# ZhengyiLuo/PHC

Measured on NVIDIA H100. Metric: env-steps/sec (fused obs+reward+PPO) at 4096 envs/GPU, higher is better.
Workload: dtype f32

## Files before the change

phc_b200/csrc/gemm_wgmma.cu:

```cuda
#include <cuda_runtime.h>
#include <stdint.h>
#include <stdlib.h>
#include <string.h>

#include "../../include/phc_b200.h"
#include "phc_common.cuh"

extern "C" void phc_set_error(const char* msg);
extern "C" int phc_check_cuda(cudaError_t e, const char* what);
extern "C" void phc_count_launches(int n);

namespace phc {
namespace wg {

constexpr int BM = 128, NUM_THREADS = 256, MAX_PROBLEMS = PHC_GEMM_GROUP_MAX;

template <int BN>
struct Cfg {
  static constexpr int BK = BN == 128 ? 32 : 16;
  static constexpr int A_TILE = BM * BK * 4;
  static constexpr int B_TILE = BN * BK * 4;
  static constexpr int STAGE = 2 * (A_TILE + B_TILE);
  static constexpr int SMEM = 2 * STAGE;
  static constexpr int SBO = BK * 32;
  static constexpr int A_PER = BM * BK / NUM_THREADS;
  static constexpr int B_PER = BN * BK / NUM_THREADS;
};

struct Prob {
  const float* A; const float* B; const float* A_lo; const float* B_lo;
  float* C; float* C_hi; float* C_lo;
  const float* bias;
  float* aux;
  long long lda, ldb, ldc, ldaux;
  int M, N, K;
  float alpha;
  int act, accumulate, a_k, b_k, k_splits;
  int tiles_m, tiles_n, kb_total, kb_per, tile_begin, tile_count;
  unsigned int* turn;
  int turn_first, turn_total;
};

struct Params {
  Prob p[MAX_PROBLEMS];
  int count, total_tiles;
  unsigned int* sched;
  int single_pass;
};

__device__ __forceinline__ void wgmma_tf32_n128(float (&d)[64], uint64_t da, uint64_t db) {
  asm volatile(
      "{\n\t.reg .pred p;\n\tsetp.ne.b32 p, 1, 0;\n\t"
      "wgmma.mma_async.sync.aligned.m64n128k8.f32.tf32.tf32 {%0, %1, %2, %3, %4, %5, %6, %7, %8, %9, %10, %11, %12, %13, %14, %15, %16, %17, %18, %19, %20, %21, %22, %23, %24, %25, %26, %27, %28, %29, %30, %31, %32, %33, %34, %35, %36, %37, %38, %39, %40, %41, %42, %43, %44, %45, %46, %47, %48, %49, %50, %51, %52, %53, %54, %55, %56, %57, %58, %59, %60, %61, %62, %63}, %64, %65, p, 1, 1;\n\t}"
      : "+f"(d[0]), "+f"(d[1]), "+f"(d[2]), "+f"(d[3]), "+f"(d[4]), "+f"(d[5]), "+f"(d[6]), "+f"(d[7]), "+f"(d[8]), "+f"(d[9]), "+f"(d[10]), "+f"(d[11]), "+f"(d[12]), "+f"(d[13]), "+f"(d[14]), "+f"(d[15]), "+f"(d[16]), "+f"(d[17]), "+f"(d[18]), "+f"(d[19]), "+f"(d[20]), "+f"(d[21]), "+f"(d[22]), "+f"(d[23]), "+f"(d[24]), "+f"(d[25]), "+f"(d[26]), "+f"(d[27]), "+f"(d[28]), "+f"(d[29]), "+f"(d[30]), "+f"(d[31]), "+f"(d[32]), "+f"(d[33]), "+f"(d[34]), "+f"(d[35]), "+f"(d[36]), "+f"(d[37]), "+f"(d[38]), "+f"(d[39]), "+f"(d[40]), "+f"(d[41]), "+f"(d[42]), "+f"(d[43]), "+f"(d[44]), "+f"(d[45]), "+f"(d[46]), "+f"(d[47]), "+f"(d[48]), "+f"(d[49]), "+f"(d[50]), "+f"(d[51]), "+f"(d[52]), "+f"(d[53]), "+f"(d[54]), "+f"(d[55]), "+f"(d[56]), "+f"(d[57]), "+f"(d[58]), "+f"(d[59]), "+f"(d[60]), "+f"(d[61]), "+f"(d[62]), "+f"(d[63])
      : "l"(da), "l"(db));
}
__device__ __forceinline__ void wgmma_tf32_n256(float (&d)[128], uint64_t da, uint64_t db) {
  asm volatile(
      "{\n\t.reg .pred p;\n\tsetp.ne.b32 p, 1, 0;\n\t"
      "wgmma.mma_async.sync.aligned.m64n256k8.f32.tf32.tf32 {%0, %1, %2, %3, %4, %5, %6, %7, %8, %9, %10, %11, %12, %13, %14, %15, %16, %17, %18, %19, %20, %21, %22, %23, %24, %25, %26, %27, %28, %29, %30, %31, %32, %33, %34, %35, %36, %37, %38, %39, %40, %41, %42, %43, %44, %45, %46, %47, %48, %49, %50, %51, %52, %53, %54, %55, %56, %57, %58, %59, %60, %61, %62, %63, %64, %65, %66, %67, %68, %69, %70, %71, %72, %73, %74, %75, %76, %77, %78, %79, %80, %81, %82, %83, %84, %85, %86, %87, %88, %89, %90, %91, %92, %93, %94, %95, %96, %97, %98, %99, %100, %101, %102, %103, %104, %105, %106, %107, %108, %109, %110, %111, %112, %113, %114, %115, %116, %117, %118, %119, %120, %121, %122, %123, %124, %125, %126, %127}, %128, %129, p, 1, 1;\n\t}"
      : "+f"(d[0]), "+f"(d[1]), "+f"(d[2]), "+f"(d[3]), "+f"(d[4]), "+f"(d[5]), "+f"(d[6]), "+f"(d[7]), "+f"(d[8]), "+f"(d[9]), "+f"(d[10]), "+f"(d[11]), "+f"(d[12]), "+f"(d[13]), "+f"(d[14]), "+f"(d[15]), "+f"(d[16]), "+f"(d[17]), "+f"(d[18]), "+f"(d[19]), "+f"(d[20]), "+f"(d[21]), "+f"(d[22]), "+f"(d[23]), "+f"(d[24]), "+f"(d[25]), "+f"(d[26]), "+f"(d[27]), "+f"(d[28]), "+f"(d[29]), "+f"(d[30]), "+f"(d[31]), "+f"(d[32]), "+f"(d[33]), "+f"(d[34]), "+f"(d[35]), "+f"(d[36]), "+f"(d[37]), "+f"(d[38]), "+f"(d[39]), "+f"(d[40]), "+f"(d[41]), "+f"(d[42]), "+f"(d[43]), "+f"(d[44]), "+f"(d[45]), "+f"(d[46]), "+f"(d[47]), "+f"(d[48]), "+f"(d[49]), "+f"(d[50]), "+f"(d[51]), "+f"(d[52]), "+f"(d[53]), "+f"(d[54]), "+f"(d[55]), "+f"(d[56]), "+f"(d[57]), "+f"(d[58]), "+f"(d[59]), "+f"(d[60]), "+f"(d[61]), "+f"(d[62]), "+f"(d[63]), "+f"(d[64]), "+f"(d[65]), "+f"(d[66]), "+f"(d[67]), "+f"(d[68]), "+f"(d[69]), "+f"(d[70]), "+f"(d[71]), "+f"(d[72]), "+f"(d[73]), "+f"(d[74]), "+f"(d[75]), "+f"(d[76]), "+f"(d[77]), "+f"(d[78]), "+f"(d[79]), "+f"(d[80]), "+f"(d[81]), "+f"(d[82]), "+f"(d[83]), "+f"(d[84]), "+f"(d[85]), "+f"(d[86]), "+f"(d[87]), "+f"(d[88]), "+f"(d[89]), "+f"(d[90]), "+f"(d[91]), "+f"(d[92]), "+f"(d[93]), "+f"(d[94]), "+f"(d[95]), "+f"(d[96]), "+f"(d[97]), "+f"(d[98]), "+f"(d[99]), "+f"(d[100]), "+f"(d[101]), "+f"(d[102]), "+f"(d[103]), "+f"(d[104]), "+f"(d[105]), "+f"(d[106]), "+f"(d[107]), "+f"(d[108]), "+f"(d[109]), "+f"(d[110]), "+f"(d[111]), "+f"(d[112]), "+f"(d[113]), "+f"(d[114]), "+f"(d[115]), "+f"(d[116]), "+f"(d[117]), "+f"(d[118]), "+f"(d[119]), "+f"(d[120]), "+f"(d[121]), "+f"(d[122]), "+f"(d[123]), "+f"(d[124]), "+f"(d[125]), "+f"(d[126]), "+f"(d[127])
      : "l"(da), "l"(db));
}

__device__ __forceinline__ void wgmma_fence() { asm volatile("wgmma.fence.sync.aligned;" ::: "memory"); }
__device__ __forceinline__ void wgmma_commit() { asm volatile("wgmma.commit_group.sync.aligned;" ::: "memory"); }
__device__ __forceinline__ void wgmma_wait_all() { asm volatile("wgmma.wait_group.sync.aligned 0;" ::: "memory"); }

__device__ __forceinline__ uint64_t smem_desc(uint32_t addr, uint32_t lbo, uint32_t sbo) {
  return (uint64_t)((addr & 0x3FFFF) >> 4) | ((uint64_t)(lbo >> 4) << 16) | ((uint64_t)(sbo >> 4) << 32);
}

template <int BN, typename Acc>
__device__ __forceinline__ void wgmma_tf32(Acc& d, uint64_t da, uint64_t db) {
  if constexpr (BN == 128) wgmma_tf32_n128(d, da, db); else wgmma_tf32_n256(d, da, db);
}

__device__ __forceinline__ float trunc_hi(float x) { return __uint_as_float(__float_as_uint(x) & 0xFFFFE000u); }
__device__ __forceinline__ float split_lo(float x) {
  const float d = x - trunc_hi(x);
  return __uint_as_float((__float_as_uint(d) + 0x1000u) & 0xFFFFE000u);
}
__device__ __forceinline__ void sts128(uint32_t addr, float a, float b, float c, float d) {
  asm volatile("st.shared.v4.f32 [%0], {%1, %2, %3, %4};" ::"r"(addr), "f"(a), "f"(b), "f"(c), "f"(d) : "memory");
}
__device__ __forceinline__ void sts32(uint32_t addr, float a) { asm volatile("st.shared.f32 [%0], %1;" ::"r"(addr), "f"(a) : "memory"); }

template <int R, int BK>
struct Map {
  static constexpr int KC = BK / 4;
  __device__ static void kmaj(int c, int& r, int& kc) { r = (c & 7) + 8 * (c / (8 * KC)); kc = (c >> 3) % KC; }
  __device__ static void mnmaj(int e, int& r, int& k, uint32_t& off) {
    const int rl = e & 7, kl = (e >> 3) & 3, e2 = e >> 5, rh = e2 % (R / 8), kh = e2 / (R / 8);
    r = rh * 8 + rl; k = kh * 4 + kl;
    off = (uint32_t)(rh * BK * 32 + kh * 128 + rl * 16 + kl * 4);
  }
};

template <int R, int BK, int PER>
__device__ __forceinline__ void load_op(float (&v)[PER], const float* __restrict__ g, long long ld, bool kmaj, int r0, int rows, int k0,
                                        int K, int tid) {
  using Mp = Map<R, BK>;
  if (kmaj) {
#pragma unroll
    for (int i = 0; i < PER / 4; ++i) {
      int r, kc;
      Mp::kmaj(tid + i * NUM_THREADS, r, kc);
      const int rr = r0 + r, kk = k0 + 4 * kc;
      const float* src = g + (long long)rr * ld + kk;
      if (rr < rows && kk + 3 < K) {
        const float4 t = *reinterpret_cast<const float4*>(src);
        v[4 * i] = t.x; v[4 * i + 1] = t.y; v[4 * i + 2] = t.z; v[4 * i + 3] = t.w;
      } else {
#pragma unroll
        for (int e = 0; e < 4; ++e) v[4 * i + e] = (rr < rows && kk + e < K) ? src[e] : 0.f;
      }
    }
  } else {
#pragma unroll
    for (int i = 0; i < PER; ++i) {
      int r, k;
      uint32_t off;
      Mp::mnmaj(tid + i * NUM_THREADS, r, k, off);
      const int rr = r0 + r, kk = k0 + k;
      v[i] = (rr < rows && kk < K) ? g[(long long)kk * ld + rr] : 0.f;
    }
  }
}

template <int R, int BK, int PER, int MODE>
__device__ __forceinline__ void store_op(const float (&v)[PER], const float (&w)[PER], uint32_t s_hi, uint32_t s_lo, bool kmaj, int tid) {
  using Mp = Map<R, BK>;
  auto hi = [](float x) { return MODE == 2 ? x : trunc_hi(x); };
  if (kmaj) {
#pragma unroll
    for (int i = 0; i < PER / 4; ++i) {
      const uint32_t off = (uint32_t)(tid + i * NUM_THREADS) * 16u;
      sts128(s_hi + off, hi(v[4 * i]), hi(v[4 * i + 1]), hi(v[4 * i + 2]), hi(v[4 * i + 3]));
      if (MODE == 0) sts128(s_lo + off, split_lo(v[4 * i]), split_lo(v[4 * i + 1]), split_lo(v[4 * i + 2]), split_lo(v[4 * i + 3]));
      if (MODE == 2) sts128(s_lo + off, w[4 * i], w[4 * i + 1], w[4 * i + 2], w[4 * i + 3]);
    }
  } else {
#pragma unroll
    for (int i = 0; i < PER; ++i) {
      int r, k;
      uint32_t off;
      Mp::mnmaj(tid + i * NUM_THREADS, r, k, off);
      sts32(s_hi + off, hi(v[i]));
      if (MODE == 0) sts32(s_lo + off, split_lo(v[i]));
      if (MODE == 2) sts32(s_lo + off, w[i]);
    }
  }
}

__device__ __forceinline__ void split_rna(float x, float& h, float& l) {
  uint32_t a, b;
  asm("cvt.rna.tf32.f32 %0, %1;" : "=r"(a) : "f"(x));
  const float res = x - __uint_as_float(a);
  asm("cvt.rna.tf32.f32 %0, %1;" : "=r"(b) : "f"(res));
  h = __uint_as_float(a); l = __uint_as_float(b);
}

template <int BN, bool PRESPLIT>
__global__ void __launch_bounds__(NUM_THREADS, 1) gemm_wgmma_kernel(const __grid_constant__ Params P) {
  using C = Cfg<BN>;
  constexpr int BK = C::BK;
  extern __shared__ __align__(128) uint8_t smem[];
  __shared__ int s_tile;
  const int tid = threadIdx.x, lane = tid & 31, wgi = tid >> 7, wq = (tid >> 5) & 3;
  const uint32_t sbase = (uint32_t)__cvta_generic_to_shared(smem);
  const bool dyn = P.sched != nullptr;
  const bool single = !PRESPLIT && P.single_pass != 0;

  for (int it = 0;; ++it) {
    int t;
    if (dyn) {
      if (tid == 0) s_tile = (int)atomicAdd(P.sched, 1u);
      __syncthreads();
      t = s_tile;
      __syncthreads();
    } else {
      t = blockIdx.x + it * gridDim.x;
    }
    if (t >= P.total_tiles) break;
    int gi = 0;
#pragma unroll 1
    while (gi + 1 < P.count && t >= P.p[gi].tile_begin + P.p[gi].tile_count) ++gi;
    const Prob& q = P.p[gi];
    const int tl = t - q.tile_begin;
    const int ni = tl % q.tiles_n, rr = tl / q.tiles_n, mi = rr % q.tiles_m, z = rr / q.tiles_m;
    const int m0 = mi * BM, n0 = ni * BN;
    const int kb_begin = z * q.kb_per;
    const int nkb = max(0, min(q.kb_total, kb_begin + q.kb_per) - kb_begin);
    if (nkb == 0) continue;
    const bool ak = q.a_k != 0, bk = q.b_k != 0;

    float acc[BN / 2];
#pragma unroll
    for (int j = 0; j < BN / 2; ++j) acc[j] = 0.f;
    float va[C::A_PER], vb[C::B_PER], wa[PRESPLIT ? C::A_PER : 1], wb[PRESPLIT ? C::B_PER : 1];
    constexpr int MODE = PRESPLIT ? 2 : 0;
    auto load = [&](int kb) {
      const int k0 = kb * BK;
      load_op<BM, BK>(va, q.A, q.lda, ak, m0, q.M, k0, q.K, tid);
      load_op<BN, BK>(vb, q.B, q.ldb, bk, n0, q.N, k0, q.K, tid);
      if constexpr (PRESPLIT) {
        load_op<BM, BK>(wa, q.A_lo, q.lda, ak, m0, q.M, k0, q.K, tid);
        load_op<BN, BK>(wb, q.B_lo, q.ldb, bk, n0, q.N, k0, q.K, tid);
      }
    };
    auto store = [&](int buf) {
      const uint32_t s = sbase + (uint32_t)(buf * C::STAGE);
      if (single) {
        store_op<BM, BK, C::A_PER, 1>(va, va, s, 0, ak, tid);
        store_op<BN, BK, C::B_PER, 1>(vb, vb, s + 2 * C::A_TILE, 0, bk, tid);
      } else if constexpr (PRESPLIT) {
        store_op<BM, BK, C::A_PER, 2>(va, wa, s, s + C::A_TILE, ak, tid);
        store_op<BN, BK, C::B_PER, 2>(vb, wb, s + 2 * C::A_TILE, s + 2 * C::A_TILE + C::B_TILE, bk, tid);
      } else {
        store_op<BM, BK, C::A_PER, MODE>(va, va, s, s + C::A_TILE, ak, tid);
        store_op<BN, BK, C::B_PER, MODE>(vb, vb, s + 2 * C::A_TILE, s + 2 * C::A_TILE + C::B_TILE, bk, tid);
      }
      fence_async_smem();
    };

    load(kb_begin);
    store(0);
    __syncthreads();
#pragma unroll 1
    for (int i = 0; i < nkb; ++i) {
      const uint32_t s = sbase + (uint32_t)((i & 1) * C::STAGE);
      const uint32_t a_hi = s + (uint32_t)(wgi * 8 * C::SBO), a_lo = a_hi + C::A_TILE;
      const uint32_t b_hi = s + 2 * C::A_TILE, b_lo = b_hi + C::B_TILE;
      wgmma_fence();
#pragma unroll
      for (int kk = 0; kk < BK / 8; ++kk) {
        const uint32_t o = (uint32_t)kk * 256u;
        const uint64_t dAh = smem_desc(a_hi + o, 128, C::SBO), dBh = smem_desc(b_hi + o, 128, C::SBO);
        if (!single) {
          wgmma_tf32<BN>(acc, smem_desc(a_lo + o, 128, C::SBO), dBh);
          wgmma_tf32<BN>(acc, dAh, smem_desc(b_lo + o, 128, C::SBO));
        }
        wgmma_tf32<BN>(acc, dAh, dBh);
      }
      wgmma_commit();
      if (i + 1 < nkb) {
        load(kb_begin + i + 1);
        store((i + 1) & 1);
      }
      wgmma_wait_all();
      __syncthreads();
    }

    const bool ordered = q.turn != nullptr;
    volatile unsigned int* turn = ordered ? q.turn + mi * q.tiles_n + ni : nullptr;
    if (ordered) {
      if (tid == 0) {
        while (*turn != (unsigned)(q.turn_first + z)) __nanosleep(64);
        __threadfence();
      }
      __syncthreads();
    }
    const int act = q.act;
    const float* bias = (q.bias && z == 0) ? q.bias : nullptr;
#pragma unroll
    for (int h = 0; h < 2; ++h) {
      const int m = m0 + wgi * 64 + wq * 16 + (lane >> 2) + 8 * h;
      const bool row_ok = m < q.M;
      float* crow = q.C + (long long)m * q.ldc;
      float* arow = (q.aux && act < PHC_ACT_RELU_BITS && row_ok) ? q.aux + (long long)m * q.ldaux : nullptr;
      uint32_t* brow = (q.aux && act >= PHC_ACT_RELU_BITS && row_ok) ? reinterpret_cast<uint32_t*>(q.aux) + (long long)m * q.ldaux : nullptr;
#pragma unroll
      for (int qc = 0; qc < BN / 32; ++qc) {
        const int nb = n0 + 32 * qc;
        if (nb >= q.N) break;
        const uint32_t mbits = (act == PHC_ACT_MASK_BITS && brow) ? brow[nb >> 5] : 0u;
        uint32_t bits = 0;
#pragma unroll
        for (int jj = 0; jj < 4; ++jj) {
          const int j = 4 * qc + jj;
          const int nl = 8 * jj + 2 * (lane & 3);
          float v[2];
#pragma unroll
          for (int c = 0; c < 2; ++c) {
            const int n = nb + nl + c;
            float x = q.alpha * acc[4 * j + 2 * h + c];
            if (bias && n < q.N) x += bias[n];
            if (act == PHC_ACT_RELU || act == PHC_ACT_RELU_BITS) x = fmaxf(x, 0.f);
            if (act == PHC_ACT_RELU_BITS) bits |= (x > 0.f ? 1u : 0u) << (nl + c);
            else if (act == PHC_ACT_MASK_BITS) x = ((mbits >> (nl + c)) & 1u) ? x : 0.f;
            else if (arow && n < q.N) {
              if (act == PHC_ACT_SILU) { arow[n] = x; x = silu_f(x); }
              else if (act == PHC_ACT_SILU_BWD) x *= silu_grad_f(arow[n]);
              else x = arow[n] > 0.f ? x : 0.f;
            } else if (act == PHC_ACT_SILU) {
              x = silu_f(x);
            }
            v[c] = x;
          }
          if (!row_ok) continue;
          const int n = nb + nl;
          if (ordered) {
            if (n < q.N) crow[n] = __ldcg(crow + n) + v[0];
            if (n + 1 < q.N) crow[n + 1] = __ldcg(crow + n + 1) + v[1];
          } else if (q.accumulate) {
            if (n < q.N) atomicAdd(crow + n, v[0]);
            if (n + 1 < q.N) atomicAdd(crow + n + 1, v[1]);
          } else if (n + 1 < q.N) {
            *reinterpret_cast<float2*>(crow + n) = make_float2(v[0], v[1]);
          } else if (n < q.N) {
            crow[n] = v[0];
          }
          if (PRESPLIT && q.C_hi) {
            float h0, l0, h1, l1;
            split_rna(v[0], h0, l0); split_rna(v[1], h1, l1);
            if (n < q.N) { q.C_hi[(long long)m * q.ldc + n] = h0; q.C_lo[(long long)m * q.ldc + n] = l0; }
            if (n + 1 < q.N) { q.C_hi[(long long)m * q.ldc + n + 1] = h1; q.C_lo[(long long)m * q.ldc + n + 1] = l1; }
          }
        }
        if (act == PHC_ACT_RELU_BITS) {
          bits |= __shfl_xor_sync(0xffffffffu, bits, 1);
          bits |= __shfl_xor_sync(0xffffffffu, bits, 2);
          if (brow && (lane & 3) == 0) brow[nb >> 5] = bits;
        }
      }
    }
    if (ordered) {
      __threadfence();
      __syncthreads();
      if (tid == 0) *turn = (q.turn_first + z + 1 == q.turn_total) ? 0u : (unsigned)(q.turn_first + z + 1);
    }
  }
  if (dyn && tid == 0 && atomicInc(P.sched + 1, gridDim.x - 1) == gridDim.x - 1) { __threadfence(); P.sched[0] = 0u; }
}

__global__ void split_lo_kernel(const float* __restrict__ x, float* __restrict__ lo, int64_t n) {
  const int64_t stride = (int64_t)gridDim.x * blockDim.x;
  for (int64_t i = (int64_t)blockIdx.x * blockDim.x + threadIdx.x; i < n; i += stride) lo[i] = split_lo(x[i]);
}

__global__ void split_tf32_kernel(const float* __restrict__ x, int64_t ldx, int64_t rows, int cols, float* __restrict__ hi,
                                  float* __restrict__ lo, int64_t ldo) {
  const int64_t total = rows * cols;
  for (int64_t i = (int64_t)blockIdx.x * blockDim.x + threadIdx.x; i < total; i += (int64_t)gridDim.x * blockDim.x) {
    const int64_t r = i / cols;
    const int c = (int)(i - r * cols);
    split_rna(x[r * ldx + c], hi[r * ldo + c], lo[r * ldo + c]);
  }
}

static int g_single_pass = 0;
static int g_tile = 0;
static int g_sched = -1;
constexpr int SCHED_SLOTS = 64;
__device__ unsigned int g_sched_counters[SCHED_SLOTS][2];
constexpr int TURN_SLOTS = 16, TURN_TILES = 8192;
__device__ unsigned int g_turns[TURN_SLOTS][TURN_TILES];

static int num_sms() {
  static int n = 0;
  if (!n) { int dev = 0; cudaGetDevice(&dev); cudaDeviceGetAttribute(&n, cudaDevAttrMultiProcessorCount, dev); if (n <= 0) n = 132; }
  return n;
}

static int add_problem(Params& P, int n, int tiles, int bn, const float* A, const float* A_lo, long long lda, int a_k, const float* B,
                       const float* B_lo, long long ldb, int b_k, float* Cm, float* C_hi, float* C_lo, long long ldc, int M, int N, int K,
                       float alpha, const float* bias, int act, float* aux, long long ldaux, int accumulate, int k_splits) {
  const int bk = bn == 128 ? Cfg<128>::BK : Cfg<256>::BK;
  Prob& q = P.p[n];
  q.A = A; q.A_lo = A_lo; q.B = B; q.B_lo = B_lo; q.C = Cm; q.C_hi = C_hi; q.C_lo = C_lo; q.bias = bias; q.aux = aux;
  q.lda = lda; q.ldb = ldb; q.ldc = ldc; q.ldaux = ldaux; q.M = M; q.N = N; q.K = K; q.alpha = alpha; q.act = act;
  q.accumulate = accumulate ? 1 : 0; q.a_k = a_k ? 1 : 0; q.b_k = b_k ? 1 : 0;
  int ks = k_splits < 1 ? 1 : k_splits;
  q.tiles_m = (M + BM - 1) / BM;
  q.tiles_n = (N + bn - 1) / bn;
  q.kb_total = (K + bk - 1) / bk;
  if (ks > q.kb_total) ks = q.kb_total;
  q.kb_per = (q.kb_total + ks - 1) / ks;
  ks = (q.kb_total + q.kb_per - 1) / q.kb_per;
  q.k_splits = ks;
  q.turn = nullptr;
  q.tile_begin = tiles;
  q.tile_count = q.tiles_m * q.tiles_n * ks;
  return q.tile_count;
}

template <int BN, bool PRESPLIT>
static int launch(Params& P, bool dynamic_sched, cudaStream_t stream) {
  int owner[MAX_PROBLEMS];
  bool ordered = false;
  int turn_tiles = 0;
  for (int i = 0; i < P.count; ++i) {
    Prob& q = P.p[i];
    owner[i] = -1;
    for (int j = 0; j < i && q.accumulate; ++j) {
      const Prob& o = P.p[j];
      if (!o.accumulate || o.C != q.C) continue;
      if (o.M != q.M || o.N != q.N || o.ldc != q.ldc) { phc_set_error("phc_gemm_group: problems accumulating into the same C must have the same shape"); return PHC_ERR_INVALID_ARG; }
      owner[i] = owner[j] >= 0 ? owner[j] : j;
      break;
    }
  }
  bool has_members[MAX_PROBLEMS] = {};
  for (int i = 0; i < P.count; ++i)
    if (owner[i] >= 0) has_members[owner[i]] = true;
  for (int i = 0; i < P.count; ++i) {
    Prob& q = P.p[i];
    q.turn_first = 0; q.turn_total = q.k_splits;
    if (q.k_splits > 1 || owner[i] >= 0 || has_members[i]) { ordered = true; if (owner[i] < 0) turn_tiles += q.tiles_m * q.tiles_n; }
  }
  if (turn_tiles > TURN_TILES) { phc_set_error("gemm: more than 8192 ordered output tiles in one launch"); return PHC_ERR_UNSUPPORTED; }
  if (ordered) {
    static unsigned int* tbase = nullptr;
    static unsigned int turn_no = 0;
    if (!tbase) {
      void* p = nullptr;
      cudaError_t es = cudaGetSymbolAddress(&p, g_turns);
      if (es != cudaSuccess) return phc_check_cuda(es, "cudaGetSymbolAddress(g_turns)");
      tbase = static_cast<unsigned int*>(p);
    }
    unsigned int* t = tbase + (size_t)(turn_no++ % TURN_SLOTS) * TURN_TILES;
    for (int i = 0; i < P.count; ++i) {
      Prob& q = P.p[i];
      if (owner[i] >= 0) {
        Prob& o = P.p[owner[i]];
        q.turn = o.turn;
        q.turn_first = o.turn_total;
        o.turn_total += q.k_splits;
      } else if (q.k_splits > 1 || has_members[i]) {
        q.turn = t; t += q.tiles_m * q.tiles_n;
      }
    }
    for (int i = 0; i < P.count; ++i)
      if (owner[i] >= 0) P.p[i].turn_total = P.p[owner[i]].turn_total;
    dynamic_sched = true;
  }
  P.sched = nullptr;
  if (dynamic_sched) {
    static unsigned int* base = nullptr;
    static unsigned int launch_no = 0;
    if (!base) {
      void* p = nullptr;
      cudaError_t es = cudaGetSymbolAddress(&p, g_sched_counters);
      if (es != cudaSuccess) return phc_check_cuda(es, "cudaGetSymbolAddress(g_sched_counters)");
      base = static_cast<unsigned int*>(p);
    }
    P.sched = base + 2 * (launch_no++ % SCHED_SLOTS);
  }
  static bool smem_set = false;
  if (!smem_set) {
    cudaError_t e = cudaFuncSetAttribute(gemm_wgmma_kernel<BN, PRESPLIT>, cudaFuncAttributeMaxDynamicSharedMemorySize, Cfg<BN>::SMEM);
    if (e != cudaSuccess) return phc_check_cuda(e, "cudaFuncSetAttribute(gemm_wgmma)");
    smem_set = true;
  }
  const int sms = num_sms();
  const unsigned grid = (unsigned)(P.total_tiles < sms ? P.total_tiles : sms);
  gemm_wgmma_kernel<BN, PRESPLIT><<<grid, NUM_THREADS, Cfg<BN>::SMEM, stream>>>(P);
  phc_count_launches(1);
  return phc_check_cuda(cudaGetLastError(), "gemm_wgmma_kernel launch");
}

}
}

static int validate_group(const PhcGemmDesc* d, int32_t count) {
  using namespace phc::wg;
  if (!d || count < 1 || count > MAX_PROBLEMS) { phc_set_error("phc_gemm_group: 1 <= count <= PHC_GEMM_GROUP_MAX problems"); return PHC_ERR_INVALID_ARG; }
  for (int i = 0; i < count; ++i) {
    const PhcGemmDesc& g = d[i];
    if (!g.A || !g.B || !g.C || g.M < 0 || g.N < 0 || g.K < 1) { phc_set_error("phc_gemm_group: bad problem (NULL operand or negative size)"); return PHC_ERR_INVALID_ARG; }
    if (g.M == 0 || g.N == 0) continue;
    if ((g.lda & 3) || (g.ldb & 3) || (g.ldc & 3)) { phc_set_error("phc_gemm_group: leading dimensions must be multiples of 4 floats (16-byte operand loads)"); return PHC_ERR_INVALID_ARG; }
    for (const void* p : {(const void*)g.A, (const void*)g.B, (const void*)g.C})
      if (reinterpret_cast<uintptr_t>(p) & 15) { phc_set_error("phc_gemm_group: A, B, C must be 16-byte aligned"); return PHC_ERR_INVALID_ARG; }
    const int ks = g.k_splits < 1 ? 1 : g.k_splits;
    if (g.act < 0 || g.act > PHC_ACT_MASK_BITS || ((g.act == PHC_ACT_SILU_BWD || g.act == PHC_ACT_MASK_BITS) && !g.aux)) { phc_set_error("phc_gemm_group: bad activation code"); return PHC_ERR_INVALID_ARG; }
    if (g.act >= PHC_ACT_RELU_BITS && g.aux && ((reinterpret_cast<uintptr_t>(g.aux) & 3) || g.ldaux < (g.N + 31) / 32)) { phc_set_error("phc_gemm_group: bit-mask aux needs ldaux >= ceil(N / 32) words"); return PHC_ERR_INVALID_ARG; }
    if (ks > 1 && (!g.accumulate || g.act || g.aux)) { phc_set_error("phc_gemm_group: split-K needs accumulate=1 and a linear epilogue"); return PHC_ERR_INVALID_ARG; }
    if (g.B_lo && (reinterpret_cast<uintptr_t>(g.B_lo) & 15)) { phc_set_error("phc_gemm_group: B_lo must be 16-byte aligned"); return PHC_ERR_INVALID_ARG; }
  }
  auto span = [](const PhcGemmDesc& g, uintptr_t& lo, uintptr_t& hi) {
    lo = reinterpret_cast<uintptr_t>(g.C);
    hi = lo + (uintptr_t)(((int64_t)g.M - 1) * g.ldc + g.N) * sizeof(float);
  };
  for (int i = 0; i < count; ++i) {
    const PhcGemmDesc& a = d[i];
    if (a.M == 0 || a.N == 0) continue;
    uintptr_t a0, a1;
    span(a, a0, a1);
    for (int j = 0; j < i; ++j) {
      const PhcGemmDesc& b = d[j];
      if (b.M == 0 || b.N == 0) continue;
      uintptr_t b0, b1;
      span(b, b0, b1);
      if (a0 >= b1 || b0 >= a1) continue;
      if (a.accumulate && b.accumulate && a.C == b.C && a.M == b.M && a.N == b.N && a.ldc == b.ldc) continue;
      phc_set_error("phc_gemm_group: two problems write overlapping C ranges (only accumulating problems on the same C with the same M, N, ldc may)");
      return PHC_ERR_INVALID_ARG;
    }
  }
  return PHC_OK;
}

extern "C" int phc_gemm_group(const PhcGemmDesc* d, int32_t count, void* stream) {
  using namespace phc::wg;
  const int vrc = validate_group(d, count);
  if (vrc != PHC_OK) return vrc;
  if (g_sched < 0) { const char* v = getenv("PHC_TC5S_SCHED"); g_sched = (v && v[0] == 's') ? 0 : 1; }
  const int bn = g_tile == 256 ? 256 : 128;
  static Params P;
  memset(&P, 0, sizeof(P));
  int tiles = 0, n = 0;
  for (int i = 0; i < count; ++i) {
    const PhcGemmDesc& g = d[i];
    if (g.M == 0 || g.N == 0) continue;
    tiles += add_problem(P, n, tiles, bn, g.A, nullptr, g.lda, g.a_kmajor, g.B, nullptr, g.ldb, g.b_kmajor, g.C, nullptr, nullptr, g.ldc,
                         g.M, g.N, g.K, g.alpha, g.bias, g.act, g.aux, g.ldaux, g.accumulate, g.k_splits);
    ++n;
  }
  if (n == 0) return PHC_OK;
  P.count = n; P.total_tiles = tiles; P.single_pass = g_single_pass;
  cudaStream_t st = static_cast<cudaStream_t>(stream);
  return bn == 256 ? launch<256, false>(P, g_sched == 1, st) : launch<128, false>(P, g_sched == 1, st);
}

extern "C" int phc_gemm_tc5s(const float* A, int64_t lda, int32_t a_kmajor, const float* B, int64_t ldb, int32_t b_kmajor, float* C,
                             int64_t ldc, int32_t M, int32_t N, int32_t K, float alpha, const float* bias, int32_t act, float* aux,
                             int64_t ldaux, int32_t accumulate, int32_t k_splits, void* stream) {
  PhcGemmDesc d;
  d.A = A; d.lda = lda; d.a_kmajor = a_kmajor; d.B = B; d.ldb = ldb; d.b_kmajor = b_kmajor; d.C = C; d.ldc = ldc;
  d.M = M; d.N = N; d.K = K; d.alpha = alpha; d.bias = bias; d.act = act; d.aux = aux; d.ldaux = ldaux;
  d.accumulate = accumulate; d.k_splits = k_splits; d.B_lo = nullptr;
  return phc_gemm_group(&d, 1, stream);
}

extern "C" int phc_gemm_tc5(const float* A_hi, const float* A_lo, int64_t lda, int32_t a_kmajor, const float* B_hi,
                            const float* B_lo, int64_t ldb, int32_t b_kmajor, float* C, float* C_hi, float* C_lo, int64_t ldc,
                            int32_t M, int32_t N, int32_t K, float alpha, const float* bias, int32_t relu, float* mask,
                            int64_t ldmask, int32_t accumulate, int32_t k_splits, void* stream) {
  using namespace phc::wg;
// ... 62 lines not shown
```

Baseline: 193,900.

## Warp-specialize TF32 wgmma GEMM with cp.async producer and mbarrier pipeline

```diff
diff --git a/phc_b200/csrc/gemm_wgmma.cu b/phc_b200/csrc/gemm_wgmma.cu
--- a/phc_b200/csrc/gemm_wgmma.cu
+++ b/phc_b200/csrc/gemm_wgmma.cu
@@ -13,18 +13,20 @@
 namespace phc {
 namespace wg {
 
-constexpr int BM = 128, NUM_THREADS = 256, MAX_PROBLEMS = PHC_GEMM_GROUP_MAX;
-
-template <int BN>
+constexpr int BM = 128, NUM_THREADS = 384, MAX_PROBLEMS = PHC_GEMM_GROUP_MAX;
+
+template <int BN, bool PRESPLIT>
 struct Cfg {
   static constexpr int BK = BN == 128 ? 32 : 16;
   static constexpr int A_TILE = BM * BK * 4;
   static constexpr int B_TILE = BN * BK * 4;
-  static constexpr int STAGE = 2 * (A_TILE + B_TILE);
-  static constexpr int SMEM = 2 * STAGE;
-  static constexpr int SBO = BK * 32;
-  static constexpr int A_PER = BM * BK / NUM_THREADS;
-  static constexpr int B_PER = BN * BK / NUM_THREADS;
+  static constexpr int STAGE = (PRESPLIT ? 2 : 1) * (A_TILE + B_TILE);
+  static constexpr int STAGES = PRESPLIT ? 2 : 4;
+  static constexpr int SPLIT = 2 * B_TILE;
+  static constexpr int SPLIT_BUFS = 3;
+  static constexpr int BARS = STAGES * STAGE + SPLIT_BUFS * SPLIT;
+  static constexpr int SMEM = 1024 + BARS + 128;
+  static_assert((2 * STAGES + 4) * 8 + 8 <= 128, "barrier area");
 };
 
 struct Prob {
@@ -47,108 +49,79 @@
   unsigned int* sched;
   int single_pass;
 };
-
-__device__ __forceinline__ void wgmma_tf32_n128(float (&d)[64], uint64_t da, uint64_t db) {
+static_assert(sizeof(Params) <= 4096, "kernel parameter space");
+
+__device__ __forceinline__ void wgmma_rs_n128(float (&d)[64], const uint32_t* a, uint64_t db) {
   asm volatile(
       "{\n\t.reg .pred p;\n\tsetp.ne.b32 p, 1, 0;\n\t"
-      "wgmma.mma_async.sync.aligned.m64n128k8.f32.tf32.tf32 {%0, %1, %2, %3, %4, %5, %6, %7, %8, %9, %10, %11, %12, %13, %14, %15, %16, %17, %18, %19, %20, %21, %22, %23, %24, %25, %26, %27, %28, %29, %30, %31, %32, %33, %34, %35, %36, %37, %38, %39, %40, %41, %42, %43, %44, %45, %46, %47, %48, %49, %50, %51, %52, %53, %54, %55, %56, %57, %58, %59, %60, %61, %62, %63}, %64, %65, p, 1, 1;\n\t}"
+      "wgmma.mma_async.sync.aligned.m64n128k8.f32.tf32.tf32 {%0, %1, %2, %3, %4, %5, %6, %7, %8, %9, %10, %11, %12, %13, %14, %15, %16, %17, %18, %19, %20, %21, %22, %23, %24, %25, %26, %27, %28, %29, %30, %31, %32, %33, %34, %35, %36, %37, %38, %39, %40, %41, %42, %43, %44, %45, %46, %47, %48, %49, %50, %51, %52, %53, %54, %55, %56, %57, %58, %59, %60, %61, %62, %63}, {%64, %65, %66, %67}, %68, p, 1, 1;\n\t}"
       : "+f"(d[0]), "+f"(d[1]), "+f"(d[2]), "+f"(d[3]), "+f"(d[4]), "+f"(d[5]), "+f"(d[6]), "+f"(d[7]), "+f"(d[8]), "+f"(d[9]), "+f"(d[10]), "+f"(d[11]), "+f"(d[12]), "+f"(d[13]), "+f"(d[14]), "+f"(d[15]), "+f"(d[16]), "+f"(d[17]), "+f"(d[18]), "+f"(d[19]), "+f"(d[20]), "+f"(d[21]), "+f"(d[22]), "+f"(d[23]), "+f"(d[24]), "+f"(d[25]), "+f"(d[26]), "+f"(d[27]), "+f"(d[28]), "+f"(d[29]), "+f"(d[30]), "+f"(d[31]), "+f"(d[32]), "+f"(d[33]), "+f"(d[34]), "+f"(d[35]), "+f"(d[36]), "+f"(d[37]), "+f"(d[38]), "+f"(d[39]), "+f"(d[40]), "+f"(d[41]), "+f"(d[42]), "+f"(d[43]), "+f"(d[44]), "+f"(d[45]), "+f"(d[46]), "+f"(d[47]), "+f"(d[48]), "+f"(d[49]), "+f"(d[50]), "+f"(d[51]), "+f"(d[52]), "+f"(d[53]), "+f"(d[54]), "+f"(d[55]), "+f"(d[56]), "+f"(d[57]), "+f"(d[58]), "+f"(d[59]), "+f"(d[60]), "+f"(d[61]), "+f"(d[62]), "+f"(d[63])
-      : "l"(da), "l"(db));
-}
-__device__ __forceinline__ void wgmma_tf32_n256(float (&d)[128], uint64_t da, uint64_t db) {
+      : "r"(a[0]), "r"(a[1]), "r"(a[2]), "r"(a[3]), "l"(db));
+}
+__device__ __forceinline__ void wgmma_rs_n256(float (&d)[128], const uint32_t* a, uint64_t db) {
   asm volatile(
       "{\n\t.reg .pred p;\n\tsetp.ne.b32 p, 1, 0;\n\t"
-      "wgmma.mma_async.sync.aligned.m64n256k8.f32.tf32.tf32 {%0, %1, %2, %3, %4, %5, %6, %7, %8, %9, %10, %11, %12, %13, %14, %15, %16, %17, %18, %19, %20, %21, %22, %23, %24, %25, %26, %27, %28, %29, %30, %31, %32, %33, %34, %35, %36, %37, %38, %39, %40, %41, %42, %43, %44, %45, %46, %47, %48, %49, %50, %51, %52, %53, %54, %55, %56, %57, %58, %59, %60, %61, %62, %63, %64, %65, %66, %67, %68, %69, %70, %71, %72, %73, %74, %75, %76, %77, %78, %79, %80, %81, %82, %83, %84, %85, %86, %87, %88, %89, %90, %91, %92, %93, %94, %95, %96, %97, %98, %99, %100, %101, %102, %103, %104, %105, %106, %107, %108, %109, %110, %111, %112, %113, %114, %115, %116, %117, %118, %119, %120, %121, %122, %123, %124, %125, %126, %127}, %128, %129, p, 1, 1;\n\t}"
+      "wgmma.mma_async.sync.aligned.m64n256k8.f32.tf32.tf32 {%0, %1, %2, %3, %4, %5, %6, %7, %8, %9, %10, %11, %12, %13, %14, %15, %16, %17, %18, %19, %20, %21, %22, %23, %24, %25, %26, %27, %28, %29, %30, %31, %32, %33, %34, %35, %36, %37, %38, %39, %40, %41, %42, %43, %44, %45, %46, %47, %48, %49, %50, %51, %52, %53, %54, %55, %56, %57, %58, %59, %60, %61, %62, %63, %64, %65, %66, %67, %68, %69, %70, %71, %72, %73, %74, %75, %76, %77, %78, %79, %80, %81, %82, %83, %84, %85, %86, %87, %88, %89, %90, %91, %92, %93, %94, %95, %96, %97, %98, %99, %100, %101, %102, %103, %104, %105, %106, %107, %108, %109, %110, %111, %112, %113, %114, %115, %116, %117, %118, %119, %120, %121, %122, %123, %124, %125, %126, %127}, {%128, %129, %130, %131}, %132, p, 1, 1;\n\t}"
       : "+f"(d[0]), "+f"(d[1]), "+f"(d[2]), "+f"(d[3]), "+f"(d[4]), "+f"(d[5]), "+f"(d[6]), "+f"(d[7]), "+f"(d[8]), "+f"(d[9]), "+f"(d[10]), "+f"(d[11]), "+f"(d[12]), "+f"(d[13]), "+f"(d[14]), "+f"(d[15]), "+f"(d[16]), "+f"(d[17]), "+f"(d[18]), "+f"(d[19]), "+f"(d[20]), "+f"(d[21]), "+f"(d[22]), "+f"(d[23]), "+f"(d[24]), "+f"(d[25]), "+f"(d[26]), "+f"(d[27]), "+f"(d[28]), "+f"(d[29]), "+f"(d[30]), "+f"(d[31]), "+f"(d[32]), "+f"(d[33]), "+f"(d[34]), "+f"(d[35]), "+f"(d[36]), "+f"(d[37]), "+f"(d[38]), "+f"(d[39]), "+f"(d[40]), "+f"(d[41]), "+f"(d[42]), "+f"(d[43]), "+f"(d[44]), "+f"(d[45]), "+f"(d[46]), "+f"(d[47]), "+f"(d[48]), "+f"(d[49]), "+f"(d[50]), "+f"(d[51]), "+f"(d[52]), "+f"(d[53]), "+f"(d[54]), "+f"(d[55]), "+f"(d[56]), "+f"(d[57]), "+f"(d[58]), "+f"(d[59]), "+f"(d[60]), "+f"(d[61]), "+f"(d[62]), "+f"(d[63]), "+f"(d[64]), "+f"(d[65]), "+f"(d[66]), "+f"(d[67]), "+f"(d[68]), "+f"(d[69]), "+f"(d[70]), "+f"(d[71]), "+f"(d[72]), "+f"(d[73]), "+f"(d[74]), "+f"(d[75]), "+f"(d[76]), "+f"(d[77]), "+f"(d[78]), "+f"(d[79]), "+f"(d[80]), "+f"(d[81]), "+f"(d[82]), "+f"(d[83]), "+f"(d[84]), "+f"(d[85]), "+f"(d[86]), "+f"(d[87]), "+f"(d[88]), "+f"(d[89]), "+f"(d[90]), "+f"(d[91]), "+f"(d[92]), "+f"(d[93]), "+f"(d[94]), "+f"(d[95]), "+f"(d[96]), "+f"(d[97]), "+f"(d[98]), "+f"(d[99]), "+f"(d[100]), "+f"(d[101]), "+f"(d[102]), "+f"(d[103]), "+f"(d[104]), "+f"(d[105]), "+f"(d[106]), "+f"(d[107]), "+f"(d[108]), "+f"(d[109]), "+f"(d[110]), "+f"(d[111]), "+f"(d[112]), "+f"(d[113]), "+f"(d[114]), "+f"(d[115]), "+f"(d[116]), "+f"(d[117]), "+f"(d[118]), "+f"(d[119]), "+f"(d[120]), "+f"(d[121]), "+f"(d[122]), "+f"(d[123]), "+f"(d[124]), "+f"(d[125]), "+f"(d[126]), "+f"(d[127])
-      : "l"(da), "l"(db));
+      : "r"(a[0]), "r"(a[1]), "r"(a[2]), "r"(a[3]), "l"(db));
+}
+template <int BN, typename Acc>
+__device__ __forceinline__ void wgmma_tf32(Acc& d, const uint32_t* a, uint64_t db) {
+  if constexpr (BN == 128) wgmma_rs_n128(d, a, db); else wgmma_rs_n256(d, a, db);
 }
 
 __device__ __forceinline__ void wgmma_fence() { asm volatile("wgmma.fence.sync.aligned;" ::: "memory"); }
 __device__ __forceinline__ void wgmma_commit() { asm volatile("wgmma.commit_group.sync.aligned;" ::: "memory"); }
-__device__ __forceinline__ void wgmma_wait_all() { asm volatile("wgmma.wait_group.sync.aligned 0;" ::: "memory"); }
-
-__device__ __forceinline__ uint64_t smem_desc(uint32_t addr, uint32_t lbo, uint32_t sbo) {
-  return (uint64_t)((addr & 0x3FFFF) >> 4) | ((uint64_t)(lbo >> 4) << 16) | ((uint64_t)(sbo >> 4) << 32);
-}
-
-template <int BN, typename Acc>
-__device__ __forceinline__ void wgmma_tf32(Acc& d, uint64_t da, uint64_t db) {
-  if constexpr (BN == 128) wgmma_tf32_n128(d, da, db); else wgmma_tf32_n256(d, da, db);
-}
+template <int N> __device__ __forceinline__ void wgmma_wait() { asm volatile("wgmma.wait_group.sync.aligned %0;" ::"n"(N) : "memory"); }
+__device__ __forceinline__ void consumers_sync() { asm volatile("bar.sync 1, 256;" ::: "memory"); }
+
+template <int RB>
+__device__ __forceinline__ uint64_t smem_desc(uint32_t addr) {
+  return (uint64_t)((addr & 0x3FFFF) >> 4) | (1ull << 16) | ((uint64_t)((8 * RB) >> 4) << 32) | ((uint64_t)(RB == 128 ? 1 : 2) << 62);
+}
+template <int RB>
+__device__ __forceinline__ uint32_t kmaj_off(int r, int k) {
+  const uint32_t o = (uint32_t)(r * RB + k * 4);
+  return o ^ (((o >> 7) & (RB / 16 - 1)) << 4);
+}
+template <int R>
+__device__ __forceinline__ uint32_t mn_off(int k, int r) { return (uint32_t)(k * R * 4) + ((uint32_t)(r * 4) ^ ((uint32_t)(k & 3) << 5)); }
 
 __device__ __forceinline__ float trunc_hi(float x) { return __uint_as_float(__float_as_uint(x) & 0xFFFFE000u); }
 __device__ __forceinline__ float split_lo(float x) {
   const float d = x - trunc_hi(x);
   return __uint_as_float((__float_as_uint(d) + 0x1000u) & 0xFFFFE000u);
 }
+__device__ __forceinline__ float lds32(uint32_t a) { float v; asm volatile("ld.shared.f32 %0, [%1];" : "=f"(v) : "r"(a) : "memory"); return v; }
+__device__ __forceinline__ float4 lds128(uint32_t a) {
+  float4 v;
+  asm volatile("ld.shared.v4.f32 {%0, %1, %2, %3}, [%4];" : "=f"(v.x), "=f"(v.y), "=f"(v.z), "=f"(v.w) : "r"(a) : "memory");
+  return v;
+}
 __device__ __forceinline__ void sts128(uint32_t addr, float a, float b, float c, float d) {
   asm volatile("st.shared.v4.f32 [%0], {%1, %2, %3, %4};" ::"r"(addr), "f"(a), "f"(b), "f"(c), "f"(d) : "memory");
 }
-__device__ __forceinline__ void sts32(uint32_t addr, float a) { asm volatile("st.shared.f32 [%0], %1;" ::"r"(addr), "f"(a) : "memory"); }
+__device__ __forceinline__ void cp_async16(uint32_t dst, const void* src, int bytes) {
+  asm volatile("cp.async.cg.shared.global [%0], [%1], 16, %2;" ::"r"(dst), "l"(src), "r"(bytes) : "memory");
+}
 
 template <int R, int BK>
-struct Map {
-  static constexpr int KC = BK / 4;
-  __device__ static void kmaj(int c, int& r, int& kc) { r = (c & 7) + 8 * (c / (8 * KC)); kc = (c >> 3) % KC; }
-  __device__ static void mnmaj(int e, int& r, int& k, uint32_t& off) {
-    const int rl = e & 7, kl = (e >> 3) & 3, e2 = e >> 5, rh = e2 % (R / 8), kh = e2 / (R / 8);
-    r = rh * 8 + rl; k = kh * 4 + kl;
-    off = (uint32_t)(rh * BK * 32 + kh * 128 + rl * 16 + kl * 4);
-  }
-};
-
-template <int R, int BK, int PER>
-__device__ __forceinline__ void load_op(float (&v)[PER], const float* __restrict__ g, long long ld, bool kmaj, int r0, int rows, int k0,
-                                        int K, int tid) {
-  using Mp = Map<R, BK>;
+__device__ __forceinline__ void load_tile(uint32_t s, const float* __restrict__ g, long long ld, bool kmaj, int r0, int rows, int k0, int K,
+                                          int pt) {
+  constexpr int PER = R * BK / 4 / 128;
   if (kmaj) {
-#pragma unroll
-    for (int i = 0; i < PER / 4; ++i) {
-      int r, kc;
-      Mp::kmaj(tid + i * NUM_THREADS, r, kc);
-      const int rr = r0 + r, kk = k0 + 4 * kc;
-      const float* src = g + (long long)rr * ld + kk;
-      if (rr < rows && kk + 3 < K) {
-        const float4 t = *reinterpret_cast<const float4*>(src);
-        v[4 * i] = t.x; v[4 * i + 1] = t.y; v[4 * i + 2] = t.z; v[4 * i + 3] = t.w;
-      } else {
-#pragma unroll
-        for (int e = 0; e < 4; ++e) v[4 * i + e] = (rr < rows && kk + e < K) ? src[e] : 0.f;
-      }
+#pragma unroll 1
+    for (int i = 0; i < PER; ++i) {
+      const int c = pt + 128 * i, r = c / (BK / 4), k = 4 * (c % (BK / 4)), rr = r0 + r, kk = k0 + k;
+      const int n = rr < rows ? max(0, min(4, K - kk)) : 0;
+      cp_async16(s + kmaj_off<BK * 4>(r, k), n ? (const void*)(g + (long long)rr * ld + kk) : (const void*)g, 4 * n);
     }
   } else {
-#pragma unroll
+#pragma unroll 1
     for (int i = 0; i < PER; ++i) {
-      int r, k;
-      uint32_t off;
-      Mp::mnmaj(tid + i * NUM_THREADS, r, k, off);
-      const int rr = r0 + r, kk = k0 + k;
-      v[i] = (rr < rows && kk < K) ? g[(long long)kk * ld + rr] : 0.f;
-    }
-  }
-}
-
-template <int R, int BK, int PER, int MODE>
-__device__ __forceinline__ void store_op(const float (&v)[PER], const float (&w)[PER], uint32_t s_hi, uint32_t s_lo, bool kmaj, int tid) {
-  using Mp = Map<R, BK>;
-  auto hi = [](float x) { return MODE == 2 ? x : trunc_hi(x); };
-  if (kmaj) {
-#pragma unroll
-    for (int i = 0; i < PER / 4; ++i) {
-      const uint32_t off = (uint32_t)(tid + i * NUM_THREADS) * 16u;
-      sts128(s_hi + off, hi(v[4 * i]), hi(v[4 * i + 1]), hi(v[4 * i + 2]), hi(v[4 * i + 3]));
-      if (MODE == 0) sts128(s_lo + off, split_lo(v[4 * i]), split_lo(v[4 * i + 1]), split_lo(v[4 * i + 2]), split_lo(v[4 * i + 3]));
-      if (MODE == 2) sts128(s_lo + off, w[4 * i], w[4 * i + 1], w[4 * i + 2], w[4 * i + 3]);
-    }
-  } else {
-#pragma unroll
-    for (int i = 0; i < PER; ++i) {
-      int r, k;
-      uint32_t off;
-      Mp::mnmaj(tid + i * NUM_THREADS, r, k, off);
-      sts32(s_hi + off, hi(v[i]));
-      if (MODE == 0) sts32(s_lo + off, split_lo(v[i]));
-      if (MODE == 2) sts32(s_lo + off, w[i]);
+      const int c = pt + 128 * i, k = c / (R / 4), r = 4 * (c % (R / 4)), rr = r0 + r, kk = k0 + k;
+      const int n = kk < K ? max(0, min(4, rows - rr)) : 0;
+      cp_async16(s + mn_off<R>(k, r), n ? (const void*)(g + (long long)kk * ld + rr) : (const void*)g, 4 * n);
     }
   }
 }
@@ -161,105 +134,183 @@
   h = __uint_as_float(a); l = __uint_as_float(b);
 }
 
-template <int BN, bool PRESPLIT>
-__global__ void __launch_bounds__(NUM_THREADS, 1) gemm_wgmma_kernel(const __grid_constant__ Params P) {
-  using C = Cfg<BN>;
-  constexpr int BK = C::BK;
-  extern __shared__ __align__(128) uint8_t smem[];
-  __shared__ int s_tile;
-  const int tid = threadIdx.x, lane = tid & 31, wgi = tid >> 7, wq = (tid >> 5) & 3;
-  const uint32_t sbase = (uint32_t)__cvta_generic_to_shared(smem);
-  const bool dyn = P.sched != nullptr;
-  const bool single = !PRESPLIT && P.single_pass != 0;
-
-  for (int it = 0;; ++it) {
-    int t;
-    if (dyn) {
-      if (tid == 0) s_tile = (int)atomicAdd(P.sched, 1u);
-      __syncthreads();
-      t = s_tile;
-      __syncthreads();
-    } else {
-      t = blockIdx.x + it * gridDim.x;
-    }
-    if (t >= P.total_tiles) break;
-    int gi = 0;
+struct TileAt {
+  int gi, mi, ni, z, kb_begin, nkb;
+  __device__ TileAt(const Params& P, int t) {
+    gi = 0;
 #pragma unroll 1
     while (gi + 1 < P.count && t >= P.p[gi].tile_begin + P.p[gi].tile_count) ++gi;
     const Prob& q = P.p[gi];
     const int tl = t - q.tile_begin;
-    const int ni = tl % q.tiles_n, rr = tl / q.tiles_n, mi = rr % q.tiles_m, z = rr / q.tiles_m;
+    ni = tl % q.tiles_n;
+    const int rr = tl / q.tiles_n;
+    mi = rr % q.tiles_m; z = rr / q.tiles_m;
+    kb_begin = z * q.kb_per;
+    nkb = max(0, min(q.kb_total, kb_begin + q.kb_per) - kb_begin);
+  }
+};
+
+template <int BN, bool PRESPLIT, bool SINGLE>
+__global__ void __launch_bounds__(NUM_THREADS, 1) gemm_wgmma_kernel(const __grid_constant__ Params P) {
+  using C = Cfg<BN, PRESPLIT>;
+  constexpr int BK = C::BK, STAGES = C::STAGES;
+  extern __shared__ __align__(1024) uint8_t smem_raw[];
+  uint8_t* smem = reinterpret_cast<uint8_t*>((reinterpret_cast<uintptr_t>(smem_raw) + 1023) & ~uintptr_t(1023));
+  const uint32_t sbase = (uint32_t)__cvta_generic_to_shared(smem);
+  uint64_t* full = reinterpret_cast<uint64_t*>(smem + C::BARS);
+  uint64_t* empty = full + STAGES;
+  uint64_t* tile_full = empty + STAGES;
+  uint64_t* tile_empty = tile_full + 2;
+  int* tile_slot = reinterpret_cast<int*>(tile_empty + 2);
+  const int tid = threadIdx.x, lane = tid & 31;
+  const bool dyn = P.sched != nullptr;
+
+  if (tid == 0) {
+    for (int s = 0; s < STAGES; ++s) { mbar_init(full + s, 128); mbar_init(empty + s, 256); }
+    for (int j = 0; j < 2; ++j) { mbar_init(tile_full + j, 1); mbar_init(tile_empty + j, 256); }
+    mbar_init_fence();
+  }
+  __syncthreads();
+
+  if (tid < 128) {
+    asm volatile("setmaxnreg.dec.sync.aligned.u32 40;");
+    uint32_t kp = 0;
+    for (int it = 0;; ++it) {
+      const int j = it & 1;
+      mbar_wait(tile_empty + j, ((it >> 1) & 1) ^ 1);
+      if (tid == 0) {
+        tile_slot[j] = dyn ? (int)atomicAdd(P.sched, 1u) : (int)(blockIdx.x + it * gridDim.x);
+        mbar_arrive(tile_full + j);
+      }
+      asm volatile("bar.sync 2, 128;" ::: "memory");
+      const int t = tile_slot[j];
+      if (t >= P.total_tiles) break;
+      const TileAt ta(P, t);
+      const Prob& q = P.p[ta.gi];
+      const int m0 = ta.mi * BM, n0 = ta.ni * BN;
+#pragma unroll 1
+      for (int i = 0; i < ta.nkb; ++i, ++kp) {
+        const uint32_t s = kp % STAGES;
+        mbar_wait(empty + s, ((kp / STAGES) & 1) ^ 1);
+        const uint32_t st = sbase + s * C::STAGE;
+        const int k0 = (ta.kb_begin + i) * BK;
+        load_tile<BM, BK>(st, q.A, q.lda, q.a_k != 0, m0, q.M, k0, q.K, tid);
+        load_tile<BN, BK>(st + C::A_TILE, q.B, q.ldb, q.b_k != 0, n0, q.N, k0, q.K, tid);
+        if constexpr (PRESPLIT) {
+          load_tile<BM, BK>(st + C::A_TILE + C::B_TILE, q.A_lo, q.lda, q.a_k != 0, m0, q.M, k0, q.K, tid);
+          load_tile<BN, BK>(st + 2 * C::A_TILE + C::B_TILE, q.B_lo, q.ldb, q.b_k != 0, n0, q.N, k0, q.K, tid);
+        }
+        asm volatile("cp.async.mbarrier.arrive.noinc.shared::cta.b64 [%0];" ::"r"(smem_u32(full + s)) : "memory");
+      }
+    }
+    if (dyn && tid == 0 && atomicInc(P.sched + 1, gridDim.x - 1) == gridDim.x - 1) { __threadfence(); P.sched[0] = 0u; }
+    asm volatile("cp.async.wait_all;" ::: "memory");
+    return;
+  }
+
+  asm volatile("setmaxnreg.inc.sync.aligned.u32 232;");
+  const int ct = tid - 128, wgi = ct >> 7, wq = (ct >> 5) & 3;
+  const uint32_t split_base = sbase + STAGES * C::STAGE;
+  uint32_t kc = 0, sb = 0;
+  constexpr int F = BK / 2;
+  for (int it = 0;; ++it) {
+    const int j = it & 1;
+    mbar_wait(tile_full + j, (it >> 1) & 1);
+    const int t = tile_slot[j];
+    mbar_arrive(tile_empty + j);
+    if (t >= P.total_tiles) break;
+    const TileAt ta(P, t);
+    if (ta.nkb == 0) continue;
+    const Prob& q = P.p[ta.gi];
+    const int mi = ta.mi, ni = ta.ni, z = ta.z, nkb = ta.nkb;
     const int m0 = mi * BM, n0 = ni * BN;
-    const int kb_begin = z * q.kb_per;
-    const int nkb = max(0, min(q.kb_total, kb_begin + q.kb_per) - kb_begin);
-    if (nkb == 0) continue;
     const bool ak = q.a_k != 0, bk = q.b_k != 0;
 
     float acc[BN / 2];
 #pragma unroll
-    for (int j = 0; j < BN / 2; ++j) acc[j] = 0.f;
-    float va[C::A_PER], vb[C::B_PER], wa[PRESPLIT ? C::A_PER : 1], wb[PRESPLIT ? C::B_PER : 1];
-    constexpr int MODE = PRESPLIT ? 2 : 0;
-    auto load = [&](int kb) {
-      const int k0 = kb * BK;
-      load_op<BM, BK>(va, q.A, q.lda, ak, m0, q.M, k0, q.K, tid);
-      load_op<BN, BK>(vb, q.B, q.ldb, bk, n0, q.N, k0, q.K, tid);
-      if constexpr (PRESPLIT) {
-        load_op<BM, BK>(wa, q.A_lo, q.lda, ak, m0, q.M, k0, q.K, tid);
-        load_op<BN, BK>(wb, q.B_lo, q.ldb, bk, n0, q.N, k0, q.K, tid);
-      }
+    for (int jj = 0; jj < BN / 2; ++jj) acc[jj] = 0.f;
+    uint32_t ah0[F], al0[F], ah1[F], al1[F];
+    auto step = [&](uint32_t (&ah)[F], uint32_t (&al)[F]) {
+      const uint32_t s = kc % STAGES;
+      mbar_wait(full + s, (kc / STAGES) & 1);
+      const uint32_t st = sbase + s * C::STAGE;
+#pragma unroll
+      for (int e = 0; e < F; ++e) {
+        const int r = wgi * 64 + wq * 16 + (lane >> 2) + 8 * (e & 1), k = 8 * (e >> 2) + (lane & 3) + 4 * ((e >> 1) & 1);
+        const uint32_t off = ak ? kmaj_off<BK * 4>(r, k) : mn_off<BM>(k, r);
+        const float x = lds32(st + off);
+        if constexpr (PRESPLIT) { ah[e] = __float_as_uint(x); al[e] = __float_as_uint(lds32(st + C::A_TILE + C::B_TILE + off)); }
+        else {
+          ah[e] = __float_as_uint(trunc_hi(x));
+          if constexpr (!SINGLE) al[e] = __float_as_uint(split_lo(x));
+        }
+      }
+      const uint32_t sp = split_base + sb * C::SPLIT;
+#pragma unroll
+      for (int i = 0; i < 4; ++i) {
+        const int c = ct + 256 * i;
+        float4 v, w;
+        uint32_t off;
+        if (bk) {
+          off = (uint32_t)c * 16u;
+          v = lds128(st + C::A_TILE + off);
+          if constexpr (PRESPLIT) w = lds128(st + 2 * C::A_TILE + C::B_TILE + off);
+        } else {
+          const int n = c % BN, k = 4 * (c / BN);
+          off = kmaj_off<BK * 4>(n, k);
+          const uint32_t b = st + C::A_TILE;
+          v = make_float4(lds32(b + mn_off<BN>(k, n)), lds32(b + mn_off<BN>(k + 1, n)), lds32(b + mn_off<BN>(k + 2, n)),
+                          lds32(b + mn_off<BN>(k + 3, n)));
+          if constexpr (PRESPLIT) {
+            const uint32_t bl = b + C::A_TILE + C::B_TILE;
+            w = make_float4(lds32(bl + mn_off<BN>(k, n)), lds32(bl + mn_off<BN>(k + 1, n)), lds32(bl + mn_off<BN>(k + 2, n)),
+                            lds32(bl + mn_off<BN>(k + 3, n)));
+          }
+        }
+        if constexpr (PRESPLIT) {
+          sts128(sp + off, v.x, v.y, v.z, v.w);
+          sts128(sp + C::B_TILE + off, w.x, w.y, w.z, w.w);
+        } else {
+          sts128(sp + off, trunc_hi(v.x), trunc_hi(v.y), trunc_hi(v.z), trunc_hi(v.w));
+          if constexpr (!SINGLE) sts128(sp + C::B_TILE + off, split_lo(v.x), split_lo(v.y), split_lo(v.z), split_lo(v.w));
+        }
+      }
+      mbar_arrive(empty + s);
+      fence_async_smem();
+      consumers_sync();
+      wgmma_fence();
+#pragma unroll
+      for (int kk = 0; kk < BK / 8; ++kk) {
+        const uint64_t dBh = smem_desc<BK * 4>(sp + kk * 32), dBl = smem_desc<BK * 4>(sp + C::B_TILE + kk * 32);
+        if constexpr (!SINGLE) {
+          wgmma_tf32<BN>(acc, al + 4 * kk, dBh);
+          wgmma_tf32<BN>(acc, ah + 4 * kk, dBl);
+        }
+        wgmma_tf32<BN>(acc, ah + 4 * kk, dBh);
+      }
+      wgmma_commit();
+      ++kc;
+      sb = sb == C::SPLIT_BUFS - 1 ? 0 : sb + 1;
     };
-    auto store = [&](int buf) {
-      const uint32_t s = sbase + (uint32_t)(buf * C::STAGE);
-      if (single) {
-        store_op<BM, BK, C::A_PER, 1>(va, va, s, 0, ak, tid);
-        store_op<BN, BK, C::B_PER, 1>(vb, vb, s + 2 * C::A_TILE, 0, bk, tid);
-      } else if constexpr (PRESPLIT) {
-        store_op<BM, BK, C::A_PER, 2>(va, wa, s, s + C::A_TILE, ak, tid);
-        store_op<BN, BK, C::B_PER, 2>(vb, wb, s + 2 * C::A_TILE, s + 2 * C::A_TILE + C::B_TILE, bk, tid);
-      } else {
-        store_op<BM, BK, C::A_PER, MODE>(va, va, s, s + C::A_TILE, ak, tid);
-        store_op<BN, BK, C::B_PER, MODE>(vb, vb, s + 2 * C::A_TILE, s + 2 * C::A_TILE + C::B_TILE, bk, tid);
-      }
-      fence_async_smem();
-    };
-
-    load(kb_begin);
-    store(0);
-    __syncthreads();
 #pragma unroll 1
-    for (int i = 0; i < nkb; ++i) {
-      const uint32_t s = sbase + (uint32_t)((i & 1) * C::STAGE);
-      const uint32_t a_hi = s + (uint32_t)(wgi * 8 * C::SBO), a_lo = a_hi + C::A_TILE;
-      const uint32_t b_hi = s + 2 * C::A_TILE, b_lo = b_hi + C::B_TILE;
-      wgmma_fence();
-#pragma unroll
-      for (int kk = 0; kk < BK / 8; ++kk) {
-        const uint32_t o = (uint32_t)kk * 256u;
-        const uint64_t dAh = smem_desc(a_hi + o, 128, C::SBO), dBh = smem_desc(b_hi + o, 128, C::SBO);
-        if (!single) {
-          wgmma_tf32<BN>(acc, smem_desc(a_lo + o, 128, C::SBO), dBh);
-          wgmma_tf32<BN>(acc, dAh, smem_desc(b_lo + o, 128, C::SBO));
-        }
-        wgmma_tf32<BN>(acc, dAh, dBh);
-      }
-      wgmma_commit();
+    for (int i = 0; i < nkb; i += 2) {
+      step(ah0, al0);
+      wgmma_wait<1>();
       if (i + 1 < nkb) {
-        load(kb_begin + i + 1);
-        store((i + 1) & 1);
-      }
-      wgmma_wait_all();
-      __syncthreads();
-    }
+        step(ah1, al1);
+        wgmma_wait<1>();
+      }
+    }
+    wgmma_wait<0>();
 
     const bool ordered = q.turn != nullptr;
     volatile unsigned int* turn = ordered ? q.turn + mi * q.tiles_n + ni : nullptr;
     if (ordered) {
-      if (tid == 0) {
+      if (ct == 0) {
         while (*turn != (unsigned)(q.turn_first + z)) __nanosleep(64);
         __threadfence();
       }
-      __syncthreads();
+      consumers_sync();
     }
     const int act = q.act;
     const float* bias = (q.bias && z == 0) ? q.bias : nullptr;
@@ -327,11 +378,10 @@
     }
     if (ordered) {
       __threadfence();
-      __syncthreads();
-      if (tid == 0) *turn = (q.turn_first + z + 1 == q.turn_total) ? 0u : (unsigned)(q.turn_first + z + 1);
-    }
-  }
-  if (dyn && tid == 0 && atomicInc(P.sched + 1, gridDim.x - 1) == gridDim.x - 1) { __threadfence(); P.sched[0] = 0u; }
+      consumers_sync();
+      if (ct == 0) *turn = (q.turn_first + z + 1 == q.turn_total) ? 0u : (unsigned)(q.turn_first + z + 1);
+    }
+  }
 }
 
 __global__ void split_lo_kernel(const float* __restrict__ x, float* __restrict__ lo, int64_t n) {
@@ -366,7 +416,7 @@
 static int add_problem(Params& P, int n, int tiles, int bn, const float* A, const float* A_lo, long long lda, int a_k, const float* B,
                        const float* B_lo, long long ldb, int b_k, float* Cm, float* C_hi, float* C_lo, long long ldc, int M, int N, int K,
                        float alpha, const float* bias, int act, float* aux, long long ldaux, int accumulate, int k_splits) {
-  const int bk = bn == 128 ? Cfg<128>::BK : Cfg<256>::BK;
+  const int bk = bn == 128 ? Cfg<128, false>::BK : Cfg<256, false>::BK;
   Prob& q = P.p[n];
   q.A = A; q.A_lo = A_lo; q.B = B; q.B_lo = B_lo; q.C = Cm; q.C_hi = C_hi; q.C_lo = C_lo; q.bias = bias; q.aux = aux;
   q.lda = lda; q.ldb = ldb; q.ldc = ldc; q.ldaux = ldaux; q.M = M; q.N = N; q.K = K; q.alpha = alpha; q.act = act;
@@ -385,6 +435,18 @@
   return q.tile_count;
 }
 
+template <int BN, bool PRESPLIT, bool SINGLE>
+static cudaError_t run_kernel(const Params& P, unsigned grid, cudaStream_t stream) {
+  static bool smem_set = false;
+  if (!smem_set) {
+    cudaError_t e = cudaFuncSetAttribute(gemm_wgmma_kernel<BN, PRESPLIT, SINGLE>, cudaFuncAttributeMaxDynamicSharedMemorySize, Cfg<BN, PRESPLIT>::SMEM);
+    if (e != cudaSuccess) return e;
+    smem_set = true;
+  }
+  gemm_wgmma_kernel<BN, PRESPLIT, SINGLE><<<grid, NUM_THREADS, Cfg<BN, PRESPLIT>::SMEM, stream>>>(P);
+  return cudaSuccess;
+}
+
 template <int BN, bool PRESPLIT>
 static int launch(Params& P, bool dynamic_sched, cudaStream_t stream) {
   int owner[MAX_PROBLEMS];
@@ -447,15 +509,12 @@
     }
     P.sched = base + 2 * (launch_no++ % SCHED_SLOTS);
   }
-  static bool smem_set = false;
-  if (!smem_set) {
-    cudaError_t e = cudaFuncSetAttribute(gemm_wgmma_kernel<BN, PRESPLIT>, cudaFuncAttributeMaxDynamicSharedMemorySize, Cfg<BN>::SMEM);
-    if (e != cudaSuccess) return phc_check_cuda(e, "cudaFuncSetAttribute(gemm_wgmma)");
-    smem_set = true;
-  }
   const int sms = num_sms();
   const unsigned grid = (unsigned)(P.total_tiles < sms ? P.total_tiles : sms);
-  gemm_wgmma_kernel<BN, PRESPLIT><<<grid, NUM_THREADS, Cfg<BN>::SMEM, stream>>>(P);
+  cudaError_t e;
+  if constexpr (PRESPLIT) e = run_kernel<BN, true, false>(P, grid, stream);
+  else e = P.single_pass ? run_kernel<BN, false, true>(P, grid, stream) : run_kernel<BN, false, false>(P, grid, stream);
+  if (e != cudaSuccess) return phc_check_cuda(e, "cudaFuncSetAttribute(gemm_wgmma)");
   phc_count_launches(1);
   return phc_check_cuda(cudaGetLastError(), "gemm_wgmma_kernel launch");
 }
```

Result: faster. 212,100 (median of 6 runs) (+9.4%).
